# pabloconrat/our_first_climate_model

Measured on NVIDIA B200. Metric: column*wavelength*layer flux updates/s (repwvl-100 RCE step), higher is better.
Workload: dtype f64

## Files before the change

our_first_climate_model_b200/csrc/rcm_capi.cu:

```cuda
#include <algorithm>
#include <cmath>
#include <cstdio>
#include <cstdlib>
#include <cstring>
#include <new>
#include <functional>
#include <string>
#include <vector>

#include "rcm_jac.cuh"
#include "rcm_fdh.cuh"
#include "rcm_lbl_diag.cuh"

#ifndef M_PI
#define M_PI 3.14159265358979323846
#endif

struct rcm_solver {
    int device = 0;
    cudaStream_t own_stream = nullptr, stream = nullptr;
    rcm_params p{};
    DevConst dc{};
    bool const_dirty = true;
    int opt_angle_cubes = 1;
// ... 31 lines not shown
    double lbl_co2_factor = 1.0;
    bool lbl_has_o3_ref = false;
    double *d_lbl_lo = nullptr, *d_lbl_hi = nullptr, *d_lbl_tau5 = nullptr, *d_lbl_h2o_ref = nullptr,
           *d_lbl_o3_ref = nullptr, *d_sH = nullptr, *d_sO = nullptr, *d_dTstat = nullptr, *d_part = nullptr;
    size_t part_cap = 0;
    double* d_lbl_tau3s = nullptr;
    size_t tau3s_cap = 0;
    unsigned char* d_tile = nullptr;
    double* d_spart = nullptr;
    unsigned* d_counter = nullptr;
    unsigned* d_multi = nullptr;
    size_t multi_cap = 0;
    int opt_multi = 1;
    size_t tile_cap = 0, spart_cap = 0;
    bool tile_vmr_valid = false;
    std::vector<double> stage;
    std::string err;
    long launches = 0;
    std::vector<std::pair<cudaEvent_t, cudaEvent_t>> ev_free, ev_used;
    cudaStream_t pipe_stream[3] = {nullptr, nullptr, nullptr};
    cudaEvent_t pipe_done[3] = {nullptr, nullptr, nullptr}, pipe_start = nullptr;
    struct HostGraph {
        cudaGraphExec_t exec = nullptr;
        SplitArgs sig{};
        const void* host[7] = {};
        const void* dev[4] = {};
        double dT_converged = 0.0;
        int ncol = 0, nchunk = 0, nkernels = 0;
        long captures = 0, replays = 0;
        bool failed = false;
    } hg;
    cudaStream_t sp_up = nullptr, sp_rt[2] = {nullptr, nullptr}, sp_down = nullptr;
    cudaEvent_t sp_prep[24] = {}, sp_rtdone[24] = {}, sp_end = nullptr;
    double kt_ms = 0.0;
    long kt_n = 0;
    unsigned char* d_diagnose = nullptr;
    size_t diagnose_bytes = 0;
    cudaStream_t dg_stream[2] = {nullptr, nullptr};
    cudaEvent_t dg_fork = nullptr, dg_join[2] = {nullptr, nullptr};
    int* h_fdh_count = nullptr;
};

namespace {

int fail(rcm_solver* s, int code, const std::string& msg) {
    if (s) s->err = msg;
    return code;
}

int cuda_fail(rcm_solver* s, cudaError_t e, const char* what) {
    return fail(s, RCM_ERR_CUDA, std::string(what) + ": " + cudaGetErrorString(e));
}

#define CU(call)                                          \
    do {                                                  \
        cudaError_t e__ = (call);                         \
        if (e__ != cudaSuccess) return cuda_fail(s, e__, #call); \
    } while (0)
// ... 213 lines not shown
    CU(dalloc(s->d_rh, n * NLAY));
    CU(dalloc(s->d_Tprev, n * NLAY));
    CU(dalloc(s->d_time, n));
    CU(dalloc(s->d_Ed, n * NLEV));
    CU(dalloc(s->d_Eu, n * NLEV));
    CU(dalloc(s->d_dE, n * NLAY));
    CU(dalloc(s->d_dt, n));
    CU(dalloc(s->d_lowpos, n * NLAY));
    s->cap = ncol;
    s->diag_steps = 0;
    s->part_cap = 0;
    s->tile_cap = s->spart_cap = 0;
    s->tile_vmr_valid = false;
    if (s->d_dTstat) cudaFree(s->d_dTstat);
    s->d_dTstat = nullptr;
    if (s->d_solar_col) cudaFree(s->d_solar_col);
    if (s->d_cloud_col) cudaFree(s->d_cloud_col);
    s->d_solar_col = s->d_cloud_col = nullptr;
    s->has_col_solar = s->has_col_cloud = false;
    return RCM_OK;
}

int ensure_diag(rcm_solver* s, int nsteps) {
    if ((size_t)nsteps <= s->diag_steps && s->d_diag) return RCM_OK;
    CU(dalloc(s->d_diag, (size_t)nsteps * s->cap * 4));
    CU(dalloc(s->d_scalars, (size_t)nsteps * 4));
    CU(dalloc(s->d_red, rcm_reduce_scratch_doubles(nsteps)));
    CU(dalloc(s->d_ticket, (size_t)nsteps));
    CU(cudaMemsetAsync(s->d_ticket, 0, (size_t)nsteps * sizeof(unsigned), s->stream));
    s->diag_steps = nsteps;
// ... 97 lines not shown
SplitGeom split_geom(const rcm_solver* s, int ncols) {
    SplitGeom g;
    g.ntiles = (ncols + 15) / 16;
    g.nitem = (s->dc.nwvl + 3) / 4;
    g.nsplit = (g.nitem + rcm_split_ipu() - 1) / rcm_split_ipu();
    return g;
}

int ensure_split(rcm_solver* s) {
    const SplitGeom g = split_geom(s, s->cap);
    const size_t tiles = (size_t)g.ntiles, need_part = tiles * g.nsplit * rcm_split_part_doubles();
    if (tiles > s->tile_cap || !s->d_tile) {
        CU(dalloc(s->d_tile, tiles * rcm_split_tile_bytes()));
        s->tile_cap = tiles;
        s->tile_vmr_valid = false;
    }
    if (need_part > s->spart_cap || !s->d_spart) {
        CU(dalloc(s->d_spart, need_part));
        s->spart_cap = need_part;
    }
    if (tiles > s->multi_cap || !s->d_multi) {
        if (s->d_multi) CU(cudaFree(s->d_multi));
        s->d_multi = nullptr;
        CU(cudaMalloc((void**)&s->d_multi, 2 * tiles * sizeof(unsigned)));
        s->multi_cap = tiles;
    }
    if (!s->d_dTstat) CU(dalloc(s->d_dTstat, (size_t)s->cap));
    if (!s->d_counter) {
        CU(dalloc(s->d_counter, (size_t)4));
        CU(cudaMemsetAsync(s->d_counter, 0, 4 * sizeof(unsigned), s->stream));
    }
    return RCM_OK;
}

SplitArgs split_args(rcm_solver* s, int col0, int ncols, int which) {
    const SplitGeom g = split_geom(s, ncols);
    const size_t o = (size_t)col0, t0 = o / 16;
    SplitArgs a{};
    a.ncol = ncols;
    a.diag_ncol = s->ncol;
    a.ntiles = g.ntiles;
    a.nsplit = g.nsplit;
// ... 61 lines not shown
        if (s->ev_used.size() >= 1024) {
            const int rc = rcm_kernel_time_ms(s, 0, nullptr, nullptr);
            if (rc != RCM_OK) return rc;
        }
    }
    return RCM_OK;
}

int split_advance(rcm_solver* s, int nsteps) {
    int st = refresh_const(s);
    if (st != RCM_OK) return st;
    st = ensure_split(s);
    if (st != RCM_OK) return st;
    const int nsm = nsm_of(s);
    const SplitArgs a = split_args(s, 0, s->ncol, 0);
    SplitColFlags f{};
    f.prep = 1;
    f.first = (s->step_index == 0);
    f.write_all_vmr = !s->tile_vmr_valid;
    CU(rcm_launch_split_col(a, f, s->stream));
    s->launches += 1;
    s->tile_vmr_valid = true;
    static const int multi_rounds = std::getenv("RCM_MULTI_ROUNDS") ? std::atoi(std::getenv("RCM_MULTI_ROUNDS")) : 24;
    const int grid1 = split_grid(s, a, nsm);
    const bool few_rounds = a.nunits < (long long)multi_rounds * grid1;
    const bool fits = (long long)a.nunits * nsteps + 2LL * grid1 < (1LL << 31);
    if (nsteps >= 2 && fits && (s->opt_multi == 2 || (s->opt_multi == 1 && few_rounds))) {
        SplitMultiArgs m{};
        m.nsteps = nsteps;
        m.done = s->d_multi;
        m.ready = s->d_multi + a.ntiles;
        CU(cudaMemsetAsync(s->d_multi, 0, 2 * (size_t)a.ntiles * sizeof(unsigned), s->stream));
        SplitArgs am = a;
        am.quota = 1 << 30;
        CU(rcm_launch_split_multi(am, m, split_grid(s, am, nsm), s->stream));
        s->launches += 1;
        return RCM_OK;
    }
    for (int k = 0; k < nsteps; ++k) {
        st = split_rt(s, a, nsm, s->stream, k < 4);
        if (st != RCM_OK) return st;
        SplitColFlags e{};
        e.finish = 1;
        e.prep = (k + 1 < nsteps);
        e.first = 0;
        e.write_out = (k + 1 == nsteps);
        e.diag_step = k;
        CU(rcm_launch_split_col(a, e, s->stream));
        s->launches += 1;
    }
    return RCM_OK;
}

int launch(rcm_solver* s, int mode, int nsteps, bool want_diag) {
    int st = refresh_const(s);
    if (st != RCM_OK) return st;
    if (mode == MODE_RT ? !s->has_spectral : !s->has_table) return fail(s, RCM_ERR_STATE, "no lookup table loaded");
    if (s->ncol <= 0) return fail(s, RCM_ERR_STATE, "no columns loaded");
    const int nsm = nsm_of(s);
    Part parts[2];
    const int nparts = plan_parts(s, s->ncol, nsm, parts);
    std::pair<cudaEvent_t, cudaEvent_t> ev;
    if (!s->ev_free.empty()) {
        ev = s->ev_free.back();
        s->ev_free.pop_back();
// ... 210 lines not shown
        return RCM_ERR_CUDA;
    }
    set_active_species(s);
    *out = s;
    return RCM_OK;
}

int rcm_destroy(rcm_solver* s) {
    if (!s) return RCM_OK;
    cudaSetDevice(s->device);
    cudaStreamSynchronize(s->stream);
    if (g_const_owner[s->device & 63] == s) g_const_owner[s->device & 63] = nullptr;
    void* ptrs[] = {s->d_coef3, s->d_xsec_file, s->d_coef, s->d_species, s->d_planck_c, s->d_planck_k, s->d_exp_tab, s->d_T, s->d_Ts, s->d_vmr, s->d_rh,
                    s->d_Tprev, s->d_time, s->d_lbl_lo, s->d_lbl_hi, s->d_lbl_tau5, s->d_lbl_h2o_ref, s->d_lbl_o3_ref, s->d_lbl_tau3s, s->d_sH, s->d_sO,
                    s->d_dTstat, s->d_part, s->d_Ed, s->d_Eu, s->d_dE, s->d_dt, s->d_diag, s->d_scalars, s->d_red, s->d_tau,
                    s->d_lowpos, s->d_solar_col, s->d_cloud_col, s->d_ticket, s->d_tile, s->d_spart, s->d_counter, s->d_multi, s->d_diagnose};
    for (void* q : ptrs)
        if (q) cudaFree(q);
    for (auto& e : s->ev_free) { cudaEventDestroy(e.first); cudaEventDestroy(e.second); }
    for (auto& e : s->ev_used) { cudaEventDestroy(e.first); cudaEventDestroy(e.second); }
    for (int i = 0; i < 3; ++i) {
        if (s->pipe_stream[i]) cudaStreamDestroy(s->pipe_stream[i]);
        if (s->pipe_done[i]) cudaEventDestroy(s->pipe_done[i]);
    }
    if (s->pipe_start) cudaEventDestroy(s->pipe_start);
    for (cudaStream_t q : {s->sp_up, s->sp_rt[0], s->sp_rt[1], s->sp_down})
        if (q) cudaStreamDestroy(q);
    for (int i = 0; i < 24; ++i) {
        if (s->sp_prep[i]) cudaEventDestroy(s->sp_prep[i]);
        if (s->sp_rtdone[i]) cudaEventDestroy(s->sp_rtdone[i]);
    }
// ... 2 lines not shown
        if (s->dg_stream[i]) cudaStreamDestroy(s->dg_stream[i]);
        if (s->dg_join[i]) cudaEventDestroy(s->dg_join[i]);
    }
    if (s->dg_fork) cudaEventDestroy(s->dg_fork);
    if (s->h_fdh_count) cudaFreeHost(s->h_fdh_count);
    if (s->hg.exec) cudaGraphExecDestroy(s->hg.exec);
    if (s->own_stream) cudaStreamDestroy(s->own_stream);
    delete s;
    return RCM_OK;
}

const char* rcm_last_error(const rcm_solver* s) { return s ? s->err.c_str() : "null solver"; }

int rcm_set_params(rcm_solver* s, const rcm_params* p) {
    if (!s || !p) return RCM_ERR_ARG;
    if (p->nangle < 1 || p->nangle > MAX_ANGLE || p->cloud_layer >= RCM_NLAYER) return fail(s, RCM_ERR_ARG, "bad params");
    unsigned old = s->p.species_mask;
    s->p = *p;
    if (old != p->species_mask) {
        s->coef_dirty = true;
        s->ncol = 0;
    }
    s->const_dirty = true;
    set_active_species(s);
    return RCM_OK;
}

int rcm_set_option(rcm_solver* s, int option, int value) {
    if (!s) return RCM_ERR_ARG;
    if (option == 0) {
        s->opt_angle_cubes = value ? 1 : 0;
        s->const_dirty = true;
        return RCM_OK;
    }
    if (option == 1) {
        s->opt_config = value;
        s->tile_vmr_valid = false;
        return RCM_OK;
    }
    if (option == 2) {
        s->opt_cplk_narrow = value ? 1 : 0;
        return RCM_OK;
    }
    if (option == 3) {
// ... 7 lines not shown
    }
    if (option == 5) {
        s->opt_path = value ? 1 : 0;
        s->tile_vmr_valid = false;
        return RCM_OK;
    }
    if (option == 6) {
        s->opt_multi = value < 0 ? 0 : value > 2 ? 2 : value;
        return RCM_OK;
    }
    return fail(s, RCM_ERR_ARG, "unknown option");
}

int rcm_set_stream(rcm_solver* s, void* cuda_stream) {
    if (!s) return RCM_ERR_ARG;
    s->stream = cuda_stream ? (cudaStream_t)cuda_stream : s->own_stream;
    return RCM_OK;
}

int rcm_synchronize(rcm_solver* s) {
    if (!s) return RCM_ERR_ARG;
    CU(cudaSetDevice(s->device));
    CU(cudaStreamSynchronize(s->stream));
    return RCM_OK;
}

int rcm_set_repwvl_table(rcm_solver* s, const double* xsec, const double* wvl, const double* weight,
                         const double* p_grid, const double* t_ref, const double* t_pert, int n_tpert, int n_species,
                         int n_wvl, int n_p) {
    if (!s || !xsec || !wvl || !weight || !p_grid || !t_ref || !t_pert) return RCM_ERR_ARG;
    if (n_tpert < 2 || n_tpert > MAX_TPERT || n_species != RCM_NSPECIES || n_wvl < 1 || n_p < 2)
        return fail(s, RCM_ERR_ARG, "unsupported table dimensions");
    CU(cudaSetDevice(s->device));
    const size_t n = (size_t)n_tpert * n_species * n_wvl * n_p;
    CU(dalloc(s->d_xsec_file, n));
    CU(cudaMemcpy(s->d_xsec_file, xsec, n * sizeof(double), cudaMemcpyHostToDevice));
    s->coef_dirty = true;
    {
        int st = rcm_set_spectral_grid(s, wvl, weight, n_wvl);
        if (st != RCM_OK) return st;
    }
    s->p_grid.assign(p_grid, p_grid + n_p);
    s->t_ref.assign(t_ref, t_ref + n_p);
    s->t_pert.assign(t_pert, t_pert + n_tpert);
    s->dc.nwvl = n_wvl;
    s->dc.n_tpert = n_tpert;
    s->dc.n_species = n_species;
    s->dc.n_p = n_p;
    for (int m = 0; m < n_tpert; ++m) s->dc.t_pert[m] = t_pert[m];
    s->has_table = true;
    s->lbl_mode = false;
    s->const_dirty = true;
    s->tau_valid = false;
    s->tau_cap = 0;
    return RCM_OK;
}

int rcm_set_spectral_grid(rcm_solver* s, const double* wvl, const double* weight, int n_wvl) {
    if (!s || !wvl || !weight || n_wvl < 1) return RCM_ERR_ARG;
    CU(cudaSetDevice(s->device));
    const double h = 6.62607e-34, c = 299792458, kB = 1.380649e-23;
    std::vector<double> pc(n_wvl), pk(n_wvl);
    double pc_max = 0.0;
    for (int i = 0; i < n_wvl; ++i) {
        const double lam = wvl[i] * 1e-9;
        pc[i] = h * c / (lam * kB);
        pk[i] = weight[i] * 2 * h * std::pow(c, 2) / std::pow(lam, 5) / 1e9;
        if (!(wvl[i] > 0.0) || !std::isfinite(pk[i])) return fail(s, RCM_ERR_ARG, "wavelengths must be positive and finite");
        pc_max = std::max(pc_max, pc[i]);
    }
    if (pc_max / 690.0 > 20.0)
        return fail(s, RCM_ERR_ARG, "wavelengths below 1043 nm are not supported (thermal solver: the Planck exponent would leave the range of the kernels' exp)");
    s->T_floor = pc_max / 690.0;
    CU(dalloc(s->d_planck_c, (size_t)n_wvl));
// ... 11 lines not shown
    s->lbl_mode = false;
    s->const_dirty = true;
    s->tau_valid = false;
    return RCM_OK;
}

int rcm_set_repwvl_table_from(rcm_solver* s, const rcm_table* t) {
    if (!s || !t) return RCM_ERR_ARG;
    return rcm_set_repwvl_table(s, t->xsec.data(), t->wvl.data(), t->weight.data(), t->p_grid.data(), t->t_ref.data(),
                                t->t_pert.data(), t->n_tpert, t->n_species, t->n_wvl, t->n_p);
}

int rcm_set_lbl_tables(rcm_solver* s, const double* wvl, const double* tau5, int nwvl, const double* h2o_ref,
                       const double* o3_ref, double co2_factor) {
    if (!s || !wvl || !tau5 || nwvl < 2 || !h2o_ref) return RCM_ERR_ARG;
    for (int i = 1; i < nwvl; ++i)
        if (!(wvl[i] > wvl[i - 1])) return fail(s, RCM_ERR_ARG, "LBL wavelengths must be strictly ascending");
    CU(cudaSetDevice(s->device));
    std::vector<double> lo(nwvl), hi(nwvl);
    for (int i = 0; i < nwvl; ++i) {
        const double dl = (i > 0) ? (wvl[i] - wvl[i - 1]) : (wvl[1] - wvl[0]);
        const double dh = (i < nwvl - 1) ? (wvl[i + 1] - wvl[i]) : (wvl[i] - wvl[i - 1]);
        lo[i] = wvl[i] - dl / 2.0;
        hi[i] = wvl[i] + dh / 2.0;
    }
    const size_t n = (size_t)nwvl;
    CU(dalloc(s->d_lbl_lo, 4 * n));
    CU(dalloc(s->d_lbl_hi, n));
    CU(dalloc(s->d_lbl_tau5, 6 * n * NLAY));
    CU(dalloc(s->d_lbl_h2o_ref, (size_t)NLAY));
// ... 30 lines not shown
    s->lbl_mode = true;
    if (s->dc.nwvl != nwvl) {
        s->has_table = s->has_spectral = false;
        s->tau_cap = 0;
    }
    s->tau_valid = false;
    s->dc.nwvl = nwvl;
    s->const_dirty = true;
    s->part_cap = 0;
    return RCM_OK;
}

int rcm_set_columns(rcm_solver* s, int ncol, const double* plevel_hPa, const double* Tlayer, const double* Tsurf,
                    const double* vmr9, const double* rel_hum) {
    if (!s || ncol <= 0 || !plevel_hPa || !Tlayer || !Tsurf || !vmr9 || !rel_hum) return RCM_ERR_ARG;
    CU(cudaSetDevice(s->device));
    int st = ensure_columns(s, ncol);
    if (st != RCM_OK) return st;
    s->ncol = ncol;
    if (!s->has_plevel || std::memcmp(s->plevel, plevel_hPa, sizeof(s->plevel)) != 0) s->coef_dirty = true;
    std::memcpy(s->plevel, plevel_hPa, sizeof(s->plevel));
    s->has_plevel = true;
    s->const_dirty = true;
    set_active_species(s);
    const size_t n = (size_t)ncol;
    s->stage.resize(n * s->nactive * NLAY);
    for (size_t c = 0; c < n; ++c)
        for (int k = 0; k < s->nactive; ++k)
            std::memcpy(&s->stage[(c * s->nactive + k) * NLAY], vmr9 + (c * RCM_NSPECIES + s->species[k]) * NLAY,
                        NLAY * sizeof(double));
// ... 2 lines not shown
    CU(cudaMemcpyAsync(s->d_Tprev, Tlayer, n * NLAY * sizeof(double), cudaMemcpyHostToDevice, s->stream));
    CU(cudaMemcpyAsync(s->d_Ts, Tsurf, n * sizeof(double), cudaMemcpyHostToDevice, s->stream));
    CU(cudaMemcpyAsync(s->d_rh, rel_hum, n * NLAY * sizeof(double), cudaMemcpyHostToDevice, s->stream));
    CU(cudaMemsetAsync(s->d_time, 0, n * sizeof(float), s->stream));
    CU(cudaStreamSynchronize(s->stream));
    s->step_index = 0;
    s->tau_valid = false;
    s->tile_vmr_valid = false;
    s->has_col_solar = s->has_col_cloud = false;
    return RCM_OK;
}

int rcm_set_column_solar(rcm_solver* s, const rcm_solar_params* sp, const double* tau_s, const double* mu_s,
                         const double* albedo, int cloud_from_tau_s, double* solar_irr_out, double* r_total_out) {
    if (!s) return RCM_ERR_ARG;
    if (s->ncol <= 0) return fail(s, RCM_ERR_STATE, "rcm_set_columns first");
    CU(cudaSetDevice(s->device));
    if (!sp) {
        s->has_col_solar = s->has_col_cloud = false;
        s->tau_valid = false;
        return RCM_OK;
    }
    if (sp->doublings < 0 || sp->doublings > 60) return fail(s, RCM_ERR_ARG, "doublings must be in 0..60");
    if (cloud_from_tau_s && s->p.cloud_layer < 0) return fail(s, RCM_ERR_ARG, "cloud_from_tau_s needs a cloud layer");
    const size_t n = (size_t)s->ncol;
    if (!s->d_solar_col) {
        CU(dalloc(s->d_solar_col, (size_t)s->cap));
        CU(dalloc(s->d_cloud_col, (size_t)s->cap));
    }
    double* d_in = nullptr;
// ... 25 lines not shown
    if (e == cudaSuccess && r_total_out)
        e = cudaMemcpyAsync(r_total_out, d_rt, n * sizeof(double), cudaMemcpyDeviceToHost, s->stream);
    if (e == cudaSuccess) e = cudaStreamSynchronize(s->stream);
    cudaFree(d_in);
    if (d_rt) cudaFree(d_rt);
    if (e != cudaSuccess) return cuda_fail(s, e, "rcm_set_column_solar");
    s->launches += 1;
    s->has_col_solar = true;
    s->has_col_cloud = cloud_from_tau_s != 0;
    s->tau_valid = false;
    return RCM_OK;
}

int rcm_update_columns(rcm_solver* s, const double* Tlayer, const double* Tsurf, const double* vmr_active) {
    if (!s) return RCM_ERR_ARG;
    if (s->ncol <= 0) return fail(s, RCM_ERR_STATE, "rcm_set_columns first");
    CU(cudaSetDevice(s->device));
    const size_t n = (size_t)s->ncol;
    if (Tlayer) CU(cudaMemcpyAsync(s->d_T, Tlayer, n * NLAY * sizeof(double), cudaMemcpyHostToDevice, s->stream));
    if (Tsurf) CU(cudaMemcpyAsync(s->d_Ts, Tsurf, n * sizeof(double), cudaMemcpyHostToDevice, s->stream));
    if (vmr_active)
        CU(cudaMemcpyAsync(s->d_vmr, vmr_active, n * s->nactive * NLAY * sizeof(double), cudaMemcpyHostToDevice, s->stream));
    if (vmr_active) s->tile_vmr_valid = false;
    s->tau_valid = false;
    return RCM_OK;
}

int rcm_set_step_index(rcm_solver* s, long step_index) {
    if (!s || step_index < 0) return RCM_ERR_ARG;
    s->step_index = step_index;
    return RCM_OK;
}

int rcm_build_tau(rcm_solver* s, double* tau_out, int* lowpos_p, int* lowpos_t) {
    if (!s) return RCM_ERR_ARG;
    if (s->lbl_mode) return fail(s, RCM_ERR_STATE, "rcm_build_tau is the repwvl read_tau: set a repwvl table after rcm_set_lbl_tables");
    if (!s->has_table || s->ncol <= 0) return fail(s, RCM_ERR_STATE, "table and columns must be loaded");
    CU(cudaSetDevice(s->device));
    int st = ensure_tau(s);
    if (st != RCM_OK) return st;
    st = launch(s, MODE_TAU, 1, false);
    if (st != RCM_OK) return st;
    const size_t n = (size_t)s->ncol;
    if (tau_out)
        CU(cudaMemcpyAsync(tau_out, s->d_tau, n * s->dc.nwvl * NLAY * sizeof(double), cudaMemcpyDeviceToHost, s->stream));
    std::vector<int> lt;
    if (lowpos_t) CU(cudaMemcpyAsync(lowpos_t, s->d_lowpos, n * NLAY * sizeof(int), cudaMemcpyDeviceToHost, s->stream));
    CU(cudaStreamSynchronize(s->stream));
    if (lowpos_p)
        for (size_t c = 0; c < n; ++c)
            for (int k = 0; k < NLAY; ++k) lowpos_p[c * NLAY + k] = s->dc.ip[NLAY - 1 - k];
    s->tau_valid = true;
    return RCM_OK;
}

int rcm_radiative_transfer(rcm_solver* s, const double* tau, double* E_down, double* E_up, double* dE) {
    if (!s) return RCM_ERR_ARG;
    if (s->lbl_mode) return fail(s, RCM_ERR_STATE, "rcm_radiative_transfer needs a repwvl spectral grid: set one after rcm_set_lbl_tables");
    if (!s->has_spectral || s->ncol <= 0) return fail(s, RCM_ERR_STATE, "spectral grid and columns must be loaded");
    CU(cudaSetDevice(s->device));
    int st = ensure_tau(s);
    if (st != RCM_OK) return st;
    const size_t n = (size_t)s->ncol;
    if (tau) {
        CU(cudaMemcpyAsync(s->d_tau, tau, n * s->dc.nwvl * NLAY * sizeof(double), cudaMemcpyHostToDevice, s->stream));
    } else if (!s->tau_valid) {
        return fail(s, RCM_ERR_STATE, "no tau: pass one or call rcm_build_tau first");
    }
    st = launch(s, MODE_RT, 1, false);
    if (st != RCM_OK) return st;
    if (E_down) CU(cudaMemcpyAsync(E_down, s->d_Ed, n * NLEV * sizeof(double), cudaMemcpyDeviceToHost, s->stream));
    if (E_up) CU(cudaMemcpyAsync(E_up, s->d_Eu, n * NLEV * sizeof(double), cudaMemcpyDeviceToHost, s->stream));
// ... 66 lines not shown
        if (s->ev_used.size() >= 1024) {
            st = rcm_kernel_time_ms(s, 0, nullptr, nullptr);
            if (st != RCM_OK) return st;
        }
        s->launches += 3;
    }
    return RCM_OK;
}

int rcm_advance_async(rcm_solver* s, int nsteps, double** d_scalars) {
    if (!s || nsteps <= 0) return RCM_ERR_ARG;
    if ((!s->has_table && !s->lbl_mode) || s->ncol <= 0) return fail(s, RCM_ERR_STATE, "table and columns must be loaded");
    CU(cudaSetDevice(s->device));
    int st = ensure_diag(s, nsteps);
    if (st != RCM_OK) return st;
    if (s->lbl_mode) {
        st = lbl_advance(s, nsteps);
        if (st != RCM_OK) return st;
        CU(rcm_launch_reduce_diag(s->d_diag, nsteps, s->ncol, s->p.dT_converged, s->d_red, s->d_ticket, s->d_scalars, s->stream));
        s->launches += 1;
        s->step_index += nsteps;
        if (d_scalars) *d_scalars = s->d_scalars;
        return RCM_OK;
    }
    st = use_split(s) ? split_advance(s, nsteps) : launch(s, MODE_STEP, nsteps, true);
    if (st != RCM_OK) return st;
    CU(rcm_launch_reduce_diag(s->d_diag, nsteps, s->ncol, s->p.dT_converged, s->d_red, s->d_ticket, s->d_scalars, s->stream));
    s->launches += 1;
    s->step_index += nsteps;
    s->tau_valid = false;
    if (d_scalars) *d_scalars = s->d_scalars;
    return RCM_OK;
}

int rcm_advance(rcm_solver* s, int nsteps, rcm_step_scalars* scalars_out) {
    int st = rcm_advance_async(s, nsteps, nullptr);
    if (st != RCM_OK) return st;
    if (scalars_out) {
        CU(cudaMemcpyAsync(scalars_out, s->d_scalars, (size_t)nsteps * sizeof(rcm_step_scalars), cudaMemcpyDeviceToHost,
                           s->stream));
// ... 628 lines not shown
        cudaError_t e = cudaMemcpy(buf.data(), arr[k].dev, arr[k].bytes, cudaMemcpyDeviceToHost);
        if (e != cudaSuccess) {
            std::fclose(f);
            return cuda_fail(s, e, "checkpoint download");
        }
        ok = std::fwrite(buf.data(), 1, arr[k].bytes, f) == arr[k].bytes;
    }
    ok = (std::fclose(f) == 0) && ok;
    return ok ? RCM_OK : fail(s, RCM_ERR_IO, std::string("short write to ") + path);
}

int rcm_load_checkpoint(rcm_solver* s, const char* path) {
    if (!s || !path) return RCM_ERR_ARG;
    CU(cudaSetDevice(s->device));
    CU(cudaStreamSynchronize(s->stream));
    FILE* f = std::fopen(path, "rb");
    if (!f) return fail(s, RCM_ERR_IO, std::string("cannot read ") + path);
    char magic[8];
    long long hdr[8];
    double plevel[RCM_NLEVEL];
    if (std::fread(magic, 1, 8, f) != 8 || std::memcmp(magic, "RCMCKPT1", 8) != 0 || std::fread(hdr, sizeof(hdr), 1, f) != 1 ||
        std::fread(plevel, sizeof(plevel), 1, f) != 1 || hdr[0] <= 0 || hdr[0] > (1LL << 30)) {
        std::fclose(f);
        return fail(s, RCM_ERR_FORMAT, std::string(path) + " is not a checkpoint of this solver");
    }
    set_active_species(s);
    if ((unsigned)hdr[2] != s->p.species_mask || (int)hdr[1] != s->nactive) {
        std::fclose(f);
        return fail(s, RCM_ERR_STATE, "checkpoint was written with another species_mask");
    }
// ... 41 lines not shown
    if (!s->has_plevel || std::memcmp(s->plevel, plevel, sizeof(plevel)) != 0) s->coef_dirty = true;
    std::memcpy(s->plevel, plevel, sizeof(plevel));
    s->has_plevel = true;
    s->const_dirty = true;
    s->step_index = (long)hdr[3];
    s->has_col_solar = hdr[4] != 0;
    s->has_col_cloud = hdr[5] != 0;
    s->tau_valid = false;
    s->tile_vmr_valid = false;
    return RCM_OK;
}

int rcm_step_host(rcm_solver* s, const double* Tlayer_in, const double* Tsurf_in, const double* vmr_active_in,
                  double* E_down, double* E_up, double* dE, double* Tlayer_out, double* Tsurf_out) {
    if (!s) return RCM_ERR_ARG;
    int max_chunks = 8;
    if (const char* e = std::getenv("RCM_PIPE_CHUNKS")) max_chunks = std::max(1, std::min(16, std::atoi(e)));
    const int nchunk = (s && !s->lbl_mode && s->has_table) ? std::min(max_chunks, s->ncol / 4096) : 0;
    if (nchunk < 2) {
        int st = rcm_update_columns(s, Tlayer_in, Tsurf_in, vmr_active_in);
        if (st != RCM_OK) return st;
        st = rcm_advance_async(s, 1, nullptr);
        if (st != RCM_OK) return st;
        return rcm_get_state(s, Tlayer_out, Tsurf_out, nullptr, nullptr, E_down, E_up, dE, nullptr);
    }
    CU(cudaSetDevice(s->device));
    int st = ensure_diag(s, 1);
    if (st != RCM_OK) return st;
    st = refresh_const(s);
    if (st != RCM_OK) return st;
// ... 130 lines not shown
```

our_first_climate_model_b200/csrc/rcm_kernels.cu:

```cuda
#include <cfloat>
#include <cstdio>

#include "rcm_kernels.cuh"
#include "rcm_diag.cuh"
#include "rcm_jac.cuh"
#include "rcm_fjac.cuh"
#include "rcm_fdh.cuh"
#include "rcm_lbl_diag.cuh"

__constant__ DevConst cst;

cudaError_t rcm_upload_const(const DevConst& c) { return cudaMemcpyToSymbol(cst, &c, sizeof(DevConst)); }

namespace {

#include "rcm_device_math.cuh"
#include "rcm_step_kernel.cuh"

__global__ void rcm_coef_kernel(const double* __restrict__ src, double* __restrict__ dst, int nt, int ns, int nw,
                                int np, int nact, const int* __restrict__ species) {
    const size_t n = (size_t)NLAY * (nt - 1) * nw * nact;
    for (size_t i = blockIdx.x * (size_t)blockDim.x + threadIdx.x; i < n; i += (size_t)gridDim.x * blockDim.x) {
        size_t r = i;
        const int k = r % nact; r /= nact;
// ... 225 lines not shown
}

cudaError_t rcm_launch_step(int mode, const StepArgs& a, int nactive, int grid, cudaStream_t st) {
    switch (mode) {
        case MODE_STEP: return launch_m<MODE_STEP>(a, nactive, grid, st);
        case MODE_TAU: return launch_m<MODE_TAU>(a, nactive, grid, st);
        case MODE_RT: return launch_m<MODE_RT>(a, nactive, grid, st);
    }
    return cudaErrorInvalidValue;
}

size_t rcm_split_tile_bytes() { return TILE_BYTES; }
size_t rcm_split_part_doubles() { return SPLIT_PART; }
int rcm_split_ipu() { return SPLIT_IPU; }

cudaError_t rcm_launch_split_col(const SplitArgs& a, const SplitColFlags& f, cudaStream_t st) {
    rcm_split_col_kernel<<<a.ntiles, SPLIT_COL_NT, 0, st>>>(a, f);
    return cudaGetLastError();
}

cudaError_t rcm_launch_split_rt(const SplitArgs& a, int grid, cudaStream_t st) {
    auto kern = a.clampk ? rcm_split_rt_kernel<true> : rcm_split_rt_kernel<false>;
    cudaError_t e = cudaFuncSetAttribute(kern, cudaFuncAttributeMaxDynamicSharedMemorySize, (int)SPLIT_SMEM);
    if (e != cudaSuccess) return e;
    kern<<<grid, SPLIT_NT, SPLIT_SMEM, st>>>(a);
    return cudaGetLastError();
}

cudaError_t rcm_launch_split_multi(const SplitArgs& a, const SplitMultiArgs& m, int grid, cudaStream_t st) {
    auto kern = a.clampk ? rcm_split_multi_kernel<true> : rcm_split_multi_kernel<false>;
    cudaError_t e = cudaFuncSetAttribute(kern, cudaFuncAttributeMaxDynamicSharedMemorySize, (int)SPLIT_SMEM);
    if (e != cudaSuccess) return e;
// ... 173 lines not shown
```

our_first_climate_model_b200/csrc/rcm_kernels.cuh:

```cuda
#ifndef RCM_KERNELS_CUH
#define RCM_KERNELS_CUH

#include <cuda_runtime.h>

#include "rcm_internal.h"

constexpr int NLAY = RCM_NLAYER;
constexpr int NLEV = RCM_NLEVEL;
constexpr int MAX_ANGLE = 64;
constexpr int MAX_TPERT = 16;
constexpr int PLK_MAX = 128;
constexpr int MAX_PAIR = 16;
constexpr int HALF = NLAY / 2;
constexpr int RCM_LBL_C = 16, RCM_LBL_NT = 128;
#ifndef RCM_EXP_LOG2
#define RCM_EXP_LOG2 10
#endif
constexpr int EXP_LOG2 = RCM_EXP_LOG2, EXP_TAB = 1 << EXP_LOG2;
constexpr int EXP_REP = (EXP_LOG2 == 7) ? 8 : 1;
#ifdef RCM_EXP_DEG_OVERRIDE
constexpr int EXP_DEG = RCM_EXP_DEG_OVERRIDE;
#else
constexpr int EXP_DEG = (EXP_LOG2 == 7) ? 3 : 2;
#endif
// ... 93 lines not shown
    const double* solar_col; const double* cloud_col;
    unsigned char* tile;
    double* part;
    double* dTstat;
    unsigned* counter;
    int quota;
};
struct SplitColFlags {
    int finish;
    int prep;
    int first;
    int write_all_vmr;
    int write_out;
    int diag_step;
};
struct SplitMultiArgs {
    int nsteps;
    unsigned* done;
    unsigned* ready;
};
size_t rcm_split_tile_bytes();
size_t rcm_split_part_doubles();
int rcm_split_ipu();
cudaError_t rcm_launch_split_col(const SplitArgs& a, const SplitColFlags& f, cudaStream_t st);
cudaError_t rcm_launch_split_rt(const SplitArgs& a, int grid, cudaStream_t st);
cudaError_t rcm_launch_split_multi(const SplitArgs& a, const SplitMultiArgs& m, int grid, cudaStream_t st);

enum { MODE_STEP = 0, MODE_TAU = 1, MODE_RT = 2 };

size_t rcm_step_smem_bytes(int C, int nactive, int nthreads);
cudaError_t rcm_upload_const(const DevConst& c);
cudaError_t rcm_launch_step(int mode, const StepArgs& a, int nactive, int grid, cudaStream_t st);
size_t rcm_reduce_scratch_doubles(int nsteps);
cudaError_t rcm_launch_reduce_diag(const double* diag, int nsteps, int ncol, double dT_converged, double* scratch,
                                   unsigned* ticket, double* scalars, cudaStream_t st);
cudaError_t rcm_launch_coef(const double* xsec_file, double* coef, int nt, int ns, int nw, int np, int nact,
                            const int* d_species, cudaStream_t st);
cudaError_t rcm_launch_coef3(const double* coef4, double* coef3, size_t nrows, cudaStream_t st);
cudaError_t rcm_launch_microbench(int which, double* out, const double* tab, long iters, int grid,
// ... 15 lines not shown
```

our_first_climate_model_b200/csrc/rcm_split_kernels.cuh:

```cuda
#pragma once

constexpr int SPLIT_C = 16, SPLIT_NT = 128, SPLIT_G = 4;
constexpr int SPLIT_IPU = 5;
constexpr int SPLIT_COL_NT = 128;

constexpr int TB_INVT = 0;
constexpr int TB_DELT = TB_INVT + TBD_LEN;
constexpr int TB_DTDP = TB_DELT + TBD_LEN;
constexpr int TB_VMR = TB_DTDP + TBD_LEN;
constexpr int TB_INVTS = TB_VMR + 5 * TBD_LEN;
constexpr int TB_CLOUD = TB_INVTS + SPLIT_C;
constexpr int TB_DOUBLES = TB_CLOUD + SPLIT_C;
constexpr int TBI_IT = 0;
constexpr int TBI_ROWSEL = TBI_IT + TBI_LEN;
constexpr int TBI_ROWOFF = TBI_ROWSEL + TBI_LEN;
constexpr int TBI_OUTSIDE = TBI_ROWOFF + NLAY * NCAND;
constexpr int TB_INTS = (TBI_OUTSIDE + 1 + 3) / 4 * 4;
constexpr int TILE_BYTES = TB_DOUBLES * 8 + TB_INTS * 4;
static_assert(TILE_BYTES % 16 == 0, "bulk copies move multiples of 16 bytes");
constexpr int ROWB3 = 16 * 8;
constexpr int ROWS3 = ROWB3 + 16;
constexpr int ROWBUF3 = NLAY * NCAND * ROWS3;
constexpr int SPLIT_PART = 2 * NLEV * SPLIT_C;

struct SplitColSmem {
    double sT[NLAY * SPLIT_C], sTh[NLAY * SPLIT_C], sPrev[NLAY * SPLIT_C], sRh[NLAY * SPLIT_C], sEd[NLEV * SPLIT_C],
        sEu[NLEV * SPLIT_C], sdE[NLAY * SPLIT_C], sdt[SPLIT_C], sTs[SPLIT_C], sSol[SPLIT_C], sStat[SPLIT_C];
    int sit[NLAY * SPLIT_C], sitmin[NLAY], sout[NLAY + 1];
};

template <bool STANDALONE>
__device__ __forceinline__ void split_col_body(const SplitArgs& a, const SplitColFlags f, const int tile, SplitColSmem& cs) {
    constexpr int C = SPLIT_C, NT = SPLIT_COL_NT, LC = NLAY * C;
    double* const sT = cs.sT; double* const sTh = cs.sTh; double* const sPrev = cs.sPrev; double* const sRh = cs.sRh;
    double* const sEd = cs.sEd; double* const sEu = cs.sEu; double* const sdE = cs.sdE; double* const sdt = cs.sdt;
    double* const sTs = cs.sTs; double* const sSol = cs.sSol; double* const sStat = cs.sStat;
    int* const sit = cs.sit; int* const sitmin = cs.sitmin; int* const sout = cs.sout;
    int extrap = 0;
    const int tid = threadIdx.x;
    const int col0 = tile * C, ncl = min(C, a.ncol - col0);
    const int nact = cst.nactive, nwvl = cst.nwvl;
    if (STANDALONE && tile == 0 && tid == 0 && a.counter) *a.counter = 0u;
    double* const tb = reinterpret_cast<double*>(a.tile + (size_t)tile * TILE_BYTES);
    int* const tbi = reinterpret_cast<int*>(tb + TB_DOUBLES);
    const bool feedback = f.prep && !f.first && a.h2o_slot >= 0;
    for (int i = tid; i < LC; i += NT) {
        const int cc = i / NLAY, l = i % NLAY;
        const size_t gi = (size_t)(col0 + (cc < ncl ? cc : 0)) * NLAY + l;
        sT[l * C + cc] = __ldcg(a.Tlayer + gi);
        if (f.prep) sPrev[l * C + cc] = __ldcg(a.Tprev + gi);
        if (feedback) sRh[l * C + cc] = a.rel_hum[gi];
    }
    if (tid < C) {
        const int col = col0 + (tid < ncl ? tid : 0);
        sTs[tid] = __ldcg(a.Tsurf + col);
        sSol[tid] = a.solar_col ? a.solar_col[col] : cst.solar_irr;
        if (f.finish) sStat[tid] = __ldcg(a.dTstat + col);
    }
    if (f.finish) {
        const double* part = a.part + (size_t)tile * a.nsplit * SPLIT_PART;
        for (int i = tid; i < SPLIT_PART; i += NT) {
            const int row = i / C;
            double sum = 0.0;
            if (row != NLAY)
                for (int sp = 0; sp < a.nsplit; ++sp) sum += __ldcg(part + (size_t)sp * SPLIT_PART + i);
            if (row < NLAY) sEd[i + C] = sum;
            else if (row == NLAY) sEd[i % C] = 0.0;
            else sEu[i - NLEV * C] = sum;
        }
    }
    __syncthreads();

    if (f.finish) {
        for (int i = tid; i < LC; i += NT) {
            const int l = i / C, cc = i % C;
            double d = sEd[l * C + cc] - sEd[(l + 1) * C + cc] + sEu[(l + 1) * C + cc] - sEu[l * C + cc];
            if (l == NLAY - 1) d += sSol[cc] + sEd[NLAY * C + cc] - sEu[NLAY * C + cc];
            sdE[i] = d;
        }
        __syncthreads();
        if (tid < C) {
            double mx = sdE[tid], mabs = 0.0;
#pragma unroll
            for (int l = 0; l < NLAY; ++l) {
                const double d = sdE[l * C + tid];
                if (mx < d) mx = d;
// ... 23 lines not shown
            if (l == NLAY - 1) {
                const double ts = Tn * cst.conv[NLAY - 1];
                sTs[cc] = ts;
                if (cc < ncl) a.Tsurf[col0 + cc] = ts;
            }
        }
        if (f.write_out) {
            for (int i = tid; i < NLEV * ncl; i += NT) {
                const int cc = i / NLEV, l = i % NLEV;
                a.E_down[(size_t)col0 * NLEV + i] = sEd[l * C + cc];
                a.E_up[(size_t)col0 * NLEV + i] = sEu[l * C + cc];
            }
            for (int i = tid; i < NLAY * ncl; i += NT) a.dE[(size_t)col0 * NLAY + i] = sdE[(i % NLAY) * C + i / NLAY];
        }
        __syncthreads();
        if (!f.prep) {
            for (int i = tid; i < NLAY * ncl; i += NT) a.Tlayer[(size_t)col0 * NLAY + i] = sT[(i % NLAY) * C + i / NLAY];
            return;
        }
    }

    auto indices = [&] {
        for (int i = tid; i < LC; i += NT) {
            const int l = i / C, cc = i % C, r = prow(l);
            const double midT = sT[i], tref = cst.tref_ip[r];
            const int it = lowerpos_t(tref, midT, cst.n_tpert);
            const double t0 = tref + cst.t_pert[it], t1 = tref + cst.t_pert[it + 1];
            extrap |= (midT < tref + cst.t_pert[0]) | (midT > tref + cst.t_pert[cst.n_tpert - 1]);
            sit[r * C + cc] = it;
            tbi[TBI_IT + tbix(r, cc)] = it;
            const double dT = (midT - t0) / (t1 - t0);
            tb[TB_DELT + tbd(r, cc)] = dT;
            tb[TB_DTDP + tbd(r, cc)] = __dmul_rn(dT, cst.delP[r]);
        }
// ... 5 lines not shown
        const int l = i / C, cc = i % C;
        const double my = sTh[i];
        int rank = 0;
#pragma unroll
        for (int l2 = 0; l2 < NLAY; ++l2) {
            const double v = sTh[l2 * C + cc];
            rank += (v > my || (v == my && l2 < l)) ? 1 : 0;
        }
        const double Tn = my / cst.conv[rank];
        sT[rank * C + cc] = Tn;
        sdE[rank * C + cc] = fabs(Tn - sPrev[rank * C + cc]);
    }
    __syncthreads();
    for (int i = tid; i < NLAY * ncl; i += NT) {
        const double v = sT[(i % NLAY) * C + i / NLAY];
        a.Tlayer[(size_t)col0 * NLAY + i] = v;
        a.Tprev[(size_t)col0 * NLAY + i] = v;
    }
    if (tid < ncl) {
        double dmax = 0.0;
#pragma unroll
        for (int l = 0; l < NLAY; ++l) dmax = fmax(dmax, sdE[l * C + tid]);
        a.dTstat[col0 + tid] = dmax;
    }
    for (int i = tid; i < nact * LC; i += NT) {
        const int cc = i % C, l = (i / C) % NLAY, sp = i / LC;
        const bool h2o = (sp == a.h2o_slot) && !f.first;
        if (!h2o && !f.write_all_vmr) continue;
        double v = 0.0;
        if (cc < ncl) {
            const size_t gi = ((size_t)(col0 + cc) * nact + sp) * NLAY + l;
            if (h2o) {
                const double Tc = sT[l * C + cc] - 273.15;
                const double e_sat = 6.1094 * exp(17.625 * Tc / (Tc + 243.04));
                v = sRh[l * C + cc] * e_sat / cst.player[l];
                a.vmr[gi] = v;
            } else {
                v = a.vmr[gi];
            }
        }
        tb[TB_VMR + sp * TBD_LEN + tbd(prow(l), cc)] = v;
    }
    if (!f.first) indices();
    for (int i = tid; i < LC; i += NT) tb[TB_INVT + tbd(prow(i / C), i % C)] = (1.0 / fmax(sT[i], a.T_floor)) * L2E64;
    if (tid < C) {
        tb[TB_INVTS + tid] = (1.0 / fmax(sTs[tid], a.T_floor)) * L2E64;
        tb[TB_CLOUD + tid] = a.cloud_col ? a.cloud_col[col0 + (tid < ncl ? tid : 0)] : cst.cloud_tau;
    }
    const int any_extrap = __syncthreads_or(extrap);
    if (tid < NLAY) {
        int mn = sit[tid * C], mx = mn;
// ... 6 lines not shown
        for (int k = 0; k < NCAND; ++k) tbi[TBI_ROWOFF + NCAND * tid + k] = (cst.ipcell[tid] + min(mn + k, cst.n_tpert - 2)) * nwvl * ROWB3;
    }
    __syncthreads();
    for (int i = tid; i < LC; i += NT) {
        const int r = i / C;
        tbi[TBI_ROWSEL + tbix(r, i % C)] = (NCAND * r + min(sit[i] - sitmin[r], NCAND - 1)) * ROWS3;
    }
    if (tid == 0) {
        int any = any_extrap;
        for (int r = 0; r < NLAY; ++r) any |= sout[r];
        tbi[TBI_OUTSIDE] = any;
    }
}

__device__ __noinline__ void split_col_body_call(const SplitArgs& a, const SplitColFlags f, const int tile, SplitColSmem& cs) {
    split_col_body<false>(a, f, tile, cs);
}

__global__ void __launch_bounds__(SPLIT_COL_NT, 8) rcm_split_col_kernel(const SplitArgs a, const SplitColFlags f) {
    __shared__ SplitColSmem cs;
    split_col_body<true>(a, f, blockIdx.x, cs);
}

__device__ __forceinline__ unsigned ld_acquire_gpu(const unsigned* p) {
    unsigned v;
    asm volatile("ld.acquire.gpu.global.u32 %0, [%1];" : "=r"(v) : "l"(p) : "memory");
    return v;
}
__device__ __forceinline__ void st_release_gpu(unsigned* p, unsigned v) {
    asm volatile("st.release.gpu.global.u32 [%0], %1;" ::"l"(p), "r"(v) : "memory");
}

__device__ __noinline__ void wait_tile_ready(const unsigned* flag, unsigned step) {
    unsigned spins = 0;
    while (ld_acquire_gpu(flag) < step) {
        __nanosleep(128);
// ... 82 lines not shown
```

Baseline: 40.17 billion.

## Speculatively prepare next step's tile in final finish kernel, skipping separate prep launch

Result: no change. 40.22 billion, median of 6 (+0.1%).

```diff
diff --git a/our_first_climate_model_b200/csrc/rcm_capi.cu b/our_first_climate_model_b200/csrc/rcm_capi.cu
--- a/our_first_climate_model_b200/csrc/rcm_capi.cu
+++ b/our_first_climate_model_b200/csrc/rcm_capi.cu
@@ -69,6 +69,8 @@
     int opt_multi = 1;
     size_t tile_cap = 0, spart_cap = 0;
     bool tile_vmr_valid = false;
+    bool prepared = false;
+    double* d_pend = nullptr;
     std::vector<double> stage;
     std::string err;
     long launches = 0;
@@ -97,6 +99,12 @@
 };
 
 namespace {
+
+void discard_prepared(rcm_solver* s) {
+    if (!s->prepared) return;
+    s->prepared = false;
+    s->tile_vmr_valid = false;
+}
 
 int fail(rcm_solver* s, int code, const std::string& msg) {
     if (s) s->err = msg;
@@ -340,6 +348,9 @@
     s->tile_vmr_valid = false;
     if (s->d_dTstat) cudaFree(s->d_dTstat);
     s->d_dTstat = nullptr;
+    if (s->d_pend) cudaFree(s->d_pend);
+    s->d_pend = nullptr;
+    discard_prepared(s);
     if (s->d_solar_col) cudaFree(s->d_solar_col);
     if (s->d_cloud_col) cudaFree(s->d_cloud_col);
     s->d_solar_col = s->d_cloud_col = nullptr;
@@ -467,6 +478,7 @@
         CU(dalloc(s->d_tile, tiles * rcm_split_tile_bytes()));
         s->tile_cap = tiles;
         s->tile_vmr_valid = false;
+        discard_prepared(s);
     }
     if (need_part > s->spart_cap || !s->d_spart) {
         CU(dalloc(s->d_spart, need_part));
@@ -479,6 +491,7 @@
         s->multi_cap = tiles;
     }
     if (!s->d_dTstat) CU(dalloc(s->d_dTstat, (size_t)s->cap));
+    if (!s->d_pend) CU(dalloc(s->d_pend, (size_t)s->cap * (2 * NLAY + 1)));
     if (!s->d_counter) {
         CU(dalloc(s->d_counter, (size_t)4));
         CU(cudaMemsetAsync(s->d_counter, 0, 4 * sizeof(unsigned), s->stream));
@@ -570,18 +583,28 @@
     if (st != RCM_OK) return st;
     const int nsm = nsm_of(s);
     const SplitArgs a = split_args(s, 0, s->ncol, 0);
-    SplitColFlags f{};
-    f.prep = 1;
-    f.first = (s->step_index == 0);
-    f.write_all_vmr = !s->tile_vmr_valid;
-    CU(rcm_launch_split_col(a, f, s->stream));
-    s->launches += 1;
-    s->tile_vmr_valid = true;
     static const int multi_rounds = std::getenv("RCM_MULTI_ROUNDS") ? std::atoi(std::getenv("RCM_MULTI_ROUNDS")) : 24;
     const int grid1 = split_grid(s, a, nsm);
     const bool few_rounds = a.nunits < (long long)multi_rounds * grid1;
     const bool fits = (long long)a.nunits * nsteps + 2LL * grid1 < (1LL << 31);
-    if (nsteps >= 2 && fits && (s->opt_multi == 2 || (s->opt_multi == 1 && few_rounds))) {
+    const bool multi = nsteps >= 2 && fits && (s->opt_multi == 2 || (s->opt_multi == 1 && few_rounds));
+    const bool prepared = s->prepared && !multi;
+    const bool prepare_next = s->opt_multi != 0;
+    s->prepared = false;
+    SplitPending pend{};
+    pend.T = s->d_pend;
+    pend.stat = s->d_pend + (size_t)s->cap * NLAY;
+    pend.h2o = s->d_pend + (size_t)s->cap * (NLAY + 1);
+    if (!prepared) {
+        SplitColFlags f{};
+        f.prep = 1;
+        f.first = (s->step_index == 0);
+        f.write_all_vmr = !s->tile_vmr_valid;
+        CU(rcm_launch_split_col(a, f, s->stream));
+        s->launches += 1;
+        s->tile_vmr_valid = true;
+    }
+    if (multi) {
         SplitMultiArgs m{};
         m.nsteps = nsteps;
         m.done = s->d_multi;
@@ -598,13 +621,16 @@
         if (st != RCM_OK) return st;
         SplitColFlags e{};
         e.finish = 1;
-        e.prep = (k + 1 < nsteps);
+        e.prep = (k + 1 < nsteps) || prepare_next;
         e.first = 0;
         e.write_out = (k + 1 == nsteps);
         e.diag_step = k;
-        CU(rcm_launch_split_col(a, e, s->stream));
+        pend.commit = (k == 0 && prepared);
+        pend.defer = (k + 1 == nsteps) && prepare_next;
+        CU(rcm_launch_split_col(a, e, s->stream, pend));
         s->launches += 1;
     }
+    s->prepared = prepare_next;
     return RCM_OK;
 }
 
@@ -845,7 +871,8 @@
     void* ptrs[] = {s->d_coef3, s->d_xsec_file, s->d_coef, s->d_species, s->d_planck_c, s->d_planck_k, s->d_exp_tab, s->d_T, s->d_Ts, s->d_vmr, s->d_rh,
                     s->d_Tprev, s->d_time, s->d_lbl_lo, s->d_lbl_hi, s->d_lbl_tau5, s->d_lbl_h2o_ref, s->d_lbl_o3_ref, s->d_lbl_tau3s, s->d_sH, s->d_sO,
                     s->d_dTstat, s->d_part, s->d_Ed, s->d_Eu, s->d_dE, s->d_dt, s->d_diag, s->d_scalars, s->d_red, s->d_tau,
-                    s->d_lowpos, s->d_solar_col, s->d_cloud_col, s->d_ticket, s->d_tile, s->d_spart, s->d_counter, s->d_multi, s->d_diagnose};
+                    s->d_lowpos, s->d_solar_col, s->d_cloud_col, s->d_ticket, s->d_tile, s->d_spart, s->d_counter, s->d_multi, s->d_diagnose,
+                    s->d_pend};
     for (void* q : ptrs)
         if (q) cudaFree(q);
     for (auto& e : s->ev_free) { cudaEventDestroy(e.first); cudaEventDestroy(e.second); }
@@ -878,6 +905,7 @@
 
 int rcm_set_params(rcm_solver* s, const rcm_params* p) {
     if (!s || !p) return RCM_ERR_ARG;
+    discard_prepared(s);
     if (p->nangle < 1 || p->nangle > MAX_ANGLE || p->cloud_layer >= RCM_NLAYER) return fail(s, RCM_ERR_ARG, "bad params");
     unsigned old = s->p.species_mask;
     s->p = *p;
@@ -892,6 +920,7 @@
 
 int rcm_set_option(rcm_solver* s, int option, int value) {
     if (!s) return RCM_ERR_ARG;
+    discard_prepared(s);
     if (option == 0) {
         s->opt_angle_cubes = value ? 1 : 0;
         s->const_dirty = true;
@@ -929,6 +958,7 @@
 
 int rcm_set_stream(rcm_solver* s, void* cuda_stream) {
     if (!s) return RCM_ERR_ARG;
+    discard_prepared(s);
     s->stream = cuda_stream ? (cudaStream_t)cuda_stream : s->own_stream;
     return RCM_OK;
 }
@@ -944,6 +974,7 @@
                          const double* p_grid, const double* t_ref, const double* t_pert, int n_tpert, int n_species,
                          int n_wvl, int n_p) {
     if (!s || !xsec || !wvl || !weight || !p_grid || !t_ref || !t_pert) return RCM_ERR_ARG;
+    discard_prepared(s);
     if (n_tpert < 2 || n_tpert > MAX_TPERT || n_species != RCM_NSPECIES || n_wvl < 1 || n_p < 2)
         return fail(s, RCM_ERR_ARG, "unsupported table dimensions");
     CU(cudaSetDevice(s->device));
@@ -973,6 +1004,7 @@
 
 int rcm_set_spectral_grid(rcm_solver* s, const double* wvl, const double* weight, int n_wvl) {
     if (!s || !wvl || !weight || n_wvl < 1) return RCM_ERR_ARG;
+    discard_prepared(s);
     CU(cudaSetDevice(s->device));
     const double h = 6.62607e-34, c = 299792458, kB = 1.380649e-23;
     std::vector<double> pc(n_wvl), pk(n_wvl);
@@ -1014,6 +1046,7 @@
 int rcm_set_lbl_tables(rcm_solver* s, const double* wvl, const double* tau5, int nwvl, const double* h2o_ref,
                        const double* o3_ref, double co2_factor) {
     if (!s || !wvl || !tau5 || nwvl < 2 || !h2o_ref) return RCM_ERR_ARG;
+    discard_prepared(s);
     for (int i = 1; i < nwvl; ++i)
         if (!(wvl[i] > wvl[i - 1])) return fail(s, RCM_ERR_ARG, "LBL wavelengths must be strictly ascending");
     CU(cudaSetDevice(s->device));
@@ -1074,6 +1107,7 @@
 int rcm_set_columns(rcm_solver* s, int ncol, const double* plevel_hPa, const double* Tlayer, const double* Tsurf,
                     const double* vmr9, const double* rel_hum) {
     if (!s || ncol <= 0 || !plevel_hPa || !Tlayer || !Tsurf || !vmr9 || !rel_hum) return RCM_ERR_ARG;
+    discard_prepared(s);
     CU(cudaSetDevice(s->device));
     int st = ensure_columns(s, ncol);
     if (st != RCM_OK) return st;
@@ -1106,6 +1140,7 @@
 int rcm_set_column_solar(rcm_solver* s, const rcm_solar_params* sp, const double* tau_s, const double* mu_s,
                          const double* albedo, int cloud_from_tau_s, double* solar_irr_out, double* r_total_out) {
     if (!s) return RCM_ERR_ARG;
+    discard_prepared(s);
     if (s->ncol <= 0) return fail(s, RCM_ERR_STATE, "rcm_set_columns first");
     CU(cudaSetDevice(s->device));
     if (!sp) {
@@ -1161,6 +1196,7 @@
 
 int rcm_update_columns(rcm_solver* s, const double* Tlayer, const double* Tsurf, const double* vmr_active) {
     if (!s) return RCM_ERR_ARG;
+    discard_prepared(s);
     if (s->ncol <= 0) return fail(s, RCM_ERR_STATE, "rcm_set_columns first");
     CU(cudaSetDevice(s->device));
     const size_t n = (size_t)s->ncol;
@@ -1175,12 +1211,14 @@
 
 int rcm_set_step_index(rcm_solver* s, long step_index) {
     if (!s || step_index < 0) return RCM_ERR_ARG;
+    discard_prepared(s);
     s->step_index = step_index;
     return RCM_OK;
 }
 
 int rcm_build_tau(rcm_solver* s, double* tau_out, int* lowpos_p, int* lowpos_t) {
     if (!s) return RCM_ERR_ARG;
+    discard_prepared(s);
     if (s->lbl_mode) return fail(s, RCM_ERR_STATE, "rcm_build_tau is the repwvl read_tau: set a repwvl table after rcm_set_lbl_tables");
     if (!s->has_table || s->ncol <= 0) return fail(s, RCM_ERR_STATE, "table and columns must be loaded");
     CU(cudaSetDevice(s->device));
@@ -1203,6 +1241,7 @@
 
 int rcm_radiative_transfer(rcm_solver* s, const double* tau, double* E_down, double* E_up, double* dE) {
     if (!s) return RCM_ERR_ARG;
+    discard_prepared(s);
     if (s->lbl_mode) return fail(s, RCM_ERR_STATE, "rcm_radiative_transfer needs a repwvl spectral grid: set one after rcm_set_lbl_tables");
     if (!s->has_spectral || s->ncol <= 0) return fail(s, RCM_ERR_STATE, "spectral grid and columns must be loaded");
     CU(cudaSetDevice(s->device));
@@ -1299,6 +1338,8 @@
     CU(cudaSetDevice(s->device));
     int st = ensure_diag(s, nsteps);
     if (st != RCM_OK) return st;
+    const bool split = !s->lbl_mode && use_split(s);
+    if (!split) discard_prepared(s);
     if (s->lbl_mode) {
         st = lbl_advance(s, nsteps);
         if (st != RCM_OK) return st;
@@ -1308,7 +1349,7 @@
         if (d_scalars) *d_scalars = s->d_scalars;
         return RCM_OK;
     }
-    st = use_split(s) ? split_advance(s, nsteps) : launch(s, MODE_STEP, nsteps, true);
+    st = split ? split_advance(s, nsteps) : launch(s, MODE_STEP, nsteps, true);
     if (st != RCM_OK) return st;
     CU(rcm_launch_reduce_diag(s->d_diag, nsteps, s->ncol, s->p.dT_converged, s->d_red, s->d_ticket, s->d_scalars, s->stream));
     s->launches += 1;
@@ -1967,6 +2008,7 @@
     if (!s || !path) return RCM_ERR_ARG;
     CU(cudaSetDevice(s->device));
     CU(cudaStreamSynchronize(s->stream));
+    discard_prepared(s);
     FILE* f = std::fopen(path, "rb");
     if (!f) return fail(s, RCM_ERR_IO, std::string("cannot read ") + path);
     char magic[8];
@@ -2038,6 +2080,7 @@
 int rcm_step_host(rcm_solver* s, const double* Tlayer_in, const double* Tsurf_in, const double* vmr_active_in,
                   double* E_down, double* E_up, double* dE, double* Tlayer_out, double* Tsurf_out) {
     if (!s) return RCM_ERR_ARG;
+    discard_prepared(s);
     int max_chunks = 8;
     if (const char* e = std::getenv("RCM_PIPE_CHUNKS")) max_chunks = std::max(1, std::min(16, std::atoi(e)));
     const int nchunk = (s && !s->lbl_mode && s->has_table) ? std::min(max_chunks, s->ncol / 4096) : 0;
diff --git a/our_first_climate_model_b200/csrc/rcm_kernels.cu b/our_first_climate_model_b200/csrc/rcm_kernels.cu
--- a/our_first_climate_model_b200/csrc/rcm_kernels.cu
+++ b/our_first_climate_model_b200/csrc/rcm_kernels.cu
@@ -263,8 +263,8 @@
 size_t rcm_split_part_doubles() { return SPLIT_PART; }
 int rcm_split_ipu() { return SPLIT_IPU; }
 
-cudaError_t rcm_launch_split_col(const SplitArgs& a, const SplitColFlags& f, cudaStream_t st) {
-    rcm_split_col_kernel<<<a.ntiles, SPLIT_COL_NT, 0, st>>>(a, f);
+cudaError_t rcm_launch_split_col(const SplitArgs& a, const SplitColFlags& f, cudaStream_t st, const SplitPending& p) {
+    rcm_split_col_kernel<<<a.ntiles, SPLIT_COL_NT, 0, st>>>(a, f, p);
     return cudaGetLastError();
 }
 
diff --git a/our_first_climate_model_b200/csrc/rcm_kernels.cuh b/our_first_climate_model_b200/csrc/rcm_kernels.cuh
--- a/our_first_climate_model_b200/csrc/rcm_kernels.cuh
+++ b/our_first_climate_model_b200/csrc/rcm_kernels.cuh
@@ -131,6 +131,13 @@
     int write_out;
     int diag_step;
 };
+struct SplitPending {
+    int defer;
+    int commit;
+    double* T;
+    double* stat;
+    double* h2o;
+};
 struct SplitMultiArgs {
     int nsteps;
     unsigned* done;
@@ -139,7 +146,7 @@
 size_t rcm_split_tile_bytes();
 size_t rcm_split_part_doubles();
 int rcm_split_ipu();
-cudaError_t rcm_launch_split_col(const SplitArgs& a, const SplitColFlags& f, cudaStream_t st);
+cudaError_t rcm_launch_split_col(const SplitArgs& a, const SplitColFlags& f, cudaStream_t st, const SplitPending& p = SplitPending{});
 cudaError_t rcm_launch_split_rt(const SplitArgs& a, int grid, cudaStream_t st);
 cudaError_t rcm_launch_split_multi(const SplitArgs& a, const SplitMultiArgs& m, int grid, cudaStream_t st);
 
diff --git a/our_first_climate_model_b200/csrc/rcm_split_kernels.cuh b/our_first_climate_model_b200/csrc/rcm_split_kernels.cuh
--- a/our_first_climate_model_b200/csrc/rcm_split_kernels.cuh
+++ b/our_first_climate_model_b200/csrc/rcm_split_kernels.cuh
@@ -30,7 +30,8 @@
 };
 
 template <bool STANDALONE>
-__device__ __forceinline__ void split_col_body(const SplitArgs& a, const SplitColFlags f, const int tile, SplitColSmem& cs) {
+__device__ __forceinline__ void split_col_body(const SplitArgs& a, const SplitColFlags f, const int tile, SplitColSmem& cs,
+                                               const SplitPending& p) {
     constexpr int C = SPLIT_C, NT = SPLIT_COL_NT, LC = NLAY * C;
     double* const sT = cs.sT; double* const sTh = cs.sTh; double* const sPrev = cs.sPrev; double* const sRh = cs.sRh;
     double* const sEd = cs.sEd; double* const sEu = cs.sEu; double* const sdE = cs.sdE; double* const sdt = cs.sdt;
@@ -44,18 +45,19 @@
     double* const tb = reinterpret_cast<double*>(a.tile + (size_t)tile * TILE_BYTES);
     int* const tbi = reinterpret_cast<int*>(tb + TB_DOUBLES);
     const bool feedback = f.prep && !f.first && a.h2o_slot >= 0;
+    const bool defer = STANDALONE && p.defer, commit = STANDALONE && p.commit;
     for (int i = tid; i < LC; i += NT) {
         const int cc = i / NLAY, l = i % NLAY;
         const size_t gi = (size_t)(col0 + (cc < ncl ? cc : 0)) * NLAY + l;
-        sT[l * C + cc] = __ldcg(a.Tlayer + gi);
-        if (f.prep) sPrev[l * C + cc] = __ldcg(a.Tprev + gi);
+        sT[l * C + cc] = __ldcg((commit ? p.T : a.Tlayer) + gi);
+        if (f.prep) sPrev[l * C + cc] = __ldcg((commit ? p.T : a.Tprev) + gi);
         if (feedback) sRh[l * C + cc] = a.rel_hum[gi];
     }
     if (tid < C) {
         const int col = col0 + (tid < ncl ? tid : 0);
         sTs[tid] = __ldcg(a.Tsurf + col);
         sSol[tid] = a.solar_col ? a.solar_col[col] : cst.solar_irr;
-        if (f.finish) sStat[tid] = __ldcg(a.dTstat + col);
+        if (f.finish) sStat[tid] = __ldcg((commit ? p.stat : a.dTstat) + col);
     }
     if (f.finish) {
         const double* part = a.part + (size_t)tile * a.nsplit * SPLIT_PART;
@@ -70,6 +72,21 @@
         }
     }
     __syncthreads();
+    if (commit) {
+        for (int i = tid; i < NLAY * ncl; i += NT) a.Tprev[(size_t)col0 * NLAY + i] = sT[(i % NLAY) * C + i / NLAY];
+        if (tid < ncl) a.dTstat[col0 + tid] = sStat[tid];
+        if (a.h2o_slot >= 0) {
+            double v[(LC + NT - 1) / NT];
+#pragma unroll
+            for (int k = 0; k < (LC + NT - 1) / NT; ++k)
+                if (tid + k * NT < NLAY * ncl) v[k] = __ldcg(p.h2o + (size_t)col0 * NLAY + tid + k * NT);
+#pragma unroll
+            for (int k = 0; k < (LC + NT - 1) / NT; ++k) {
+                const int i = tid + k * NT;
+                if (i < NLAY * ncl) a.vmr[((size_t)(col0 + i / NLAY) * nact + a.h2o_slot) * NLAY + i % NLAY] = v[k];
+            }
+        }
+    }
 
     if (f.finish) {
         for (int i = tid; i < LC; i += NT) {
@@ -123,10 +140,9 @@
             for (int i = tid; i < NLAY * ncl; i += NT) a.dE[(size_t)col0 * NLAY + i] = sdE[(i % NLAY) * C + i / NLAY];
         }
         __syncthreads();
-        if (!f.prep) {
+        if (!f.prep || defer)
             for (int i = tid; i < NLAY * ncl; i += NT) a.Tlayer[(size_t)col0 * NLAY + i] = sT[(i % NLAY) * C + i / NLAY];
-            return;
-        }
+        if (!f.prep) return;
     }
 
     auto indices = [&] {
@@ -162,14 +178,18 @@
     __syncthreads();
     for (int i = tid; i < NLAY * ncl; i += NT) {
         const double v = sT[(i % NLAY) * C + i / NLAY];
-        a.Tlayer[(size_t)col0 * NLAY + i] = v;
-        a.Tprev[(size_t)col0 * NLAY + i] = v;
+        if (defer) {
+            p.T[(size_t)col0 * NLAY + i] = v;
+        } else {
+            a.Tlayer[(size_t)col0 * NLAY + i] = v;
+            a.Tprev[(size_t)col0 * NLAY + i] = v;
+        }
     }
     if (tid < ncl) {
         double dmax = 0.0;
 #pragma unroll
         for (int l = 0; l < NLAY; ++l) dmax = fmax(dmax, sdE[l * C + tid]);
-        a.dTstat[col0 + tid] = dmax;
+        (defer ? p.stat : a.dTstat)[col0 + tid] = dmax;
     }
     for (int i = tid; i < nact * LC; i += NT) {
         const int cc = i % C, l = (i / C) % NLAY, sp = i / LC;
@@ -182,7 +202,8 @@
                 const double Tc = sT[l * C + cc] - 273.15;
                 const double e_sat = 6.1094 * exp(17.625 * Tc / (Tc + 243.04));
                 v = sRh[l * C + cc] * e_sat / cst.player[l];
-                a.vmr[gi] = v;
+                if (defer) p.h2o[(size_t)(col0 + cc) * NLAY + l] = v;
+                else a.vmr[gi] = v;
             } else {
                 v = a.vmr[gi];
             }
@@ -219,12 +240,12 @@
 }
 
 __device__ __noinline__ void split_col_body_call(const SplitArgs& a, const SplitColFlags f, const int tile, SplitColSmem& cs) {
-    split_col_body<false>(a, f, tile, cs);
-}
-
-__global__ void __launch_bounds__(SPLIT_COL_NT, 8) rcm_split_col_kernel(const SplitArgs a, const SplitColFlags f) {
+    split_col_body<false>(a, f, tile, cs, SplitPending{});
+}
+
+__global__ void __launch_bounds__(SPLIT_COL_NT, 8) rcm_split_col_kernel(const SplitArgs a, const SplitColFlags f, const SplitPending p) {
     __shared__ SplitColSmem cs;
-    split_col_body<true>(a, f, blockIdx.x, cs);
+    split_col_body<true>(a, f, blockIdx.x, cs, p);
 }
 
 __device__ __forceinline__ unsigned ld_acquire_gpu(const unsigned* p) {
```
